# ShuvalovIvan/RayTracingProject

Hardware: AMD Instinct MI355X
Metric: Mrays/sec + frame time, random-spheres 1920x1080x256spp (higher is better)
Workload: dtype f32

## Files before the change

### raytracingproject_amd/build.py

```python
from __future__ import annotations

import os
import subprocess
from concurrent.futures import ThreadPoolExecutor
from pathlib import Path

PKG = Path(__file__).resolve().parent
ROOT = PKG.parent
CSRC = PKG / "csrc"
OBJ = PKG / "build"
LIB = PKG / "lib" / "librt_hip.so"
ARCH = os.environ.get("RT_OFFLOAD_ARCH", "gfx950")
HIPCC = os.environ.get("HIPCC", "/opt/rocm/bin/hipcc")

COMMON = ["-x", "hip", f"--offload-arch={ARCH}", "-O3", "-std=c++17", "-fPIC", "-Wall",
          "-Wno-unused-function", f"-I{ROOT / 'include'}"] + os.environ.get("RT_HIPCC_EXTRA", "").split()
UNITS = {
    "rt_render_f32.hip": ["-fno-hip-fp32-correctly-rounded-divide-sqrt", "-fgpu-flush-denormals-to-zero",
                          os.environ.get("RT_F32_CONTRACT", "-ffp-contract=on")],
    "rt_render_f64.hip": ["-ffp-contract=off"],
    "rt_abi.cpp": ["-ffp-contract=off"],
    "rt_plan.cpp": ["-ffp-contract=off"],
    "rt_pack.cpp": ["-ffp-contract=off"],
    "rt_bvh.cpp": ["-ffp-contract=off"],
    "rt_obj.cpp": ["-ffp-contract=off"],
    "rt_lbvh.hip": ["-ffp-contract=off"],
    "rt_comm.cpp": [],
}
HEADERS = ["rt_device.h", "rt_render_impl.h", "rt_occluded.h", "rt_scene.h", "rt_launch.h", "rt_bvh.h", "rt_lbvh.h", "rt_ctx.h",
           "rt_treelet.h", "rt_pack.h"]


def _stale(target: Path, deps: list[Path]) -> bool:
    if not target.exists():
        return True
    t = target.stat().st_mtime
    return any(d.stat().st_mtime > t for d in deps)


def _present(p: Path) -> bool:
    try:
        return p.exists()
    except OSError:
        return False


def _compile(src: str, extra: list[str], verbose: bool) -> Path:
    obj = OBJ / (src.rsplit(".", 1)[0] + ".o")
    deps = [CSRC / src] + [CSRC / h for h in HEADERS] + [ROOT / "include" / "rt_hip.h", Path(__file__)]
    if _stale(obj, deps):
        cmd = [HIPCC, *COMMON, *extra, "-c", str(CSRC / src), "-o", str(obj)]
        if verbose:
            print(" ".join(cmd), flush=True)
        subprocess.run(cmd, check=True)
    return obj


def build_native(verbose: bool = False) -> Path:
    OBJ.mkdir(parents=True, exist_ok=True)
    LIB.parent.mkdir(parents=True, exist_ok=True)
    with ThreadPoolExecutor(max_workers=4) as ex:
        objs = list(ex.map(lambda kv: _compile(kv[0], kv[1], verbose), UNITS.items()))
    if _stale(LIB, objs):
# ... 82 lines not shown
BOXES_EXE = OBJ / "san" / "bvh_boxes_driver"


def build_bvh_boxes(verbose: bool = False) -> Path:
    BOXES_EXE.parent.mkdir(parents=True, exist_ok=True)
    srcs = [ROOT / "tests" / "cpp" / "bvh_boxes_driver.cpp", CSRC / "rt_bvh.cpp"]
    deps = srcs + [CSRC / "rt_bvh.h", CSRC / "rt_scene.h", ROOT / "include" / "rt_hip.h", Path(__file__)]
    if _stale(BOXES_EXE, deps):
        cmd = ["g++", "-std=c++17", *SAN_FLAGS, "-ffp-contract=off", f"-I{ROOT / 'include'}", *map(str, srcs), "-o",
               str(BOXES_EXE), "-lm"]
        if verbose:
            print(" ".join(cmd), flush=True)
        subprocess.run(cmd, check=True)
    return BOXES_EXE


PACK_EXE = OBJ / "san" / "pack_driver"


def build_pack(verbose: bool = False) -> Path:
    PACK_EXE.parent.mkdir(parents=True, exist_ok=True)
    srcs = [ROOT / "tests" / "cpp" / "pack_driver.cpp", CSRC / "rt_pack.cpp", CSRC / "rt_bvh.cpp"]
    deps = srcs + [CSRC / "rt_pack.h", CSRC / "rt_bvh.h", CSRC / "rt_scene.h", ROOT / "include" / "rt_hip.h",
                   Path(__file__)]
    if _stale(PACK_EXE, deps):
        cmd = ["g++", "-std=c++17", *SAN_FLAGS, "-ffp-contract=off", f"-I{ROOT / 'include'}", *map(str, srcs), "-o",
               str(PACK_EXE), "-lm"]
        if verbose:
            print(" ".join(cmd), flush=True)
        subprocess.run(cmd, check=True)
    return PACK_EXE


def build_oracle(verbose: bool = False) -> None:
    oracle = ROOT / "oracle"
    out = None if verbose else subprocess.DEVNULL
    subprocess.run(["make", "-C", str(oracle), "liboracle.so", "rt_oracle_cli", "ref-if-present"], check=True,
                   stdout=out)


if __name__ == "__main__":
    import sys
    if "--sanitize" in sys.argv[1:]:
        print(build_sanitize(verbose=True))
        sys.exit(0)
    print(build_native(verbose=True))
    print(build_dropin(verbose=True))
    build_oracle(verbose=True)
```

### raytracingproject_amd/csrc/rt_abi.cpp

```cpp
#include <hip/hip_runtime.h>

#include <algorithm>
#include <array>
#include <cmath>
#include <cstdarg>
#include <limits>
#include <cstdio>
#include <cstdlib>
#include <cstring>
#include <string>
#include <vector>

#include "../../include/rt_hip.h"
#include "rt_bvh.h"
#include "rt_device.h"
#include "rt_launch.h"
#include "rt_lbvh.h"
#include "rt_ctx.h"

using namespace rtx;
using namespace rtx_abi;


namespace {
// ... 104 lines not shown
    int n = 0;
    if (hipGetDeviceCount(&n) != hipSuccess) return 0;
    return n;
}

const char* rt_error_string(int code) {
    switch (code) {
        case RT_OK: return "ok";
        case RT_ERR_INVALID: return "invalid argument";
        case RT_ERR_HIP: return "HIP runtime error";
        case RT_ERR_NO_SCENE: return "no scene uploaded";
        case RT_ERR_LIMIT: return "scene or image exceeds kernel limits";
        case RT_ERR_COMM: return "RCCL error";
        default: return "unknown error";
    }
}

static bool parse_grid_suspend(const char* s, int& lanes, int& iters) {
    if (!s || !*s) return true;
    int l = 0, i = 0, n = 0;
    if (sscanf(s, "%d,%d%n", &l, &i, &n) == 2 && !s[n] && l >= 1 && l <= 64 && i >= 1 && i <= 65535) {
        lanes = l;
        iters = i;
        return true;
    }
    if (s[0] == '0' && !s[1]) {
        lanes = 0;
        iters = 0x7fffffff;
        return true;
    }
    return false;
}

rt_ctx* rt_create(int device, uint64_t seed, int precision) {
    if (precision != RT_PREC_F32 && precision != RT_PREC_F64) return nullptr;
    int n = 0;
    if (hipGetDeviceCount(&n) != hipSuccess || device < 0 || device >= n) return nullptr;
    if (hipSetDevice(device) != hipSuccess) return nullptr;
    rt_ctx* c = new rt_ctx();
    if (!parse_grid_suspend(getenv("RT_GRID_SUSPEND"), c->gsus_lanes, c->gsus_iters)) {
        fprintf(stderr, "rt_create: RT_GRID_SUSPEND must be \"0\" or \"LANES,ITERS\" (1..64, 1..65535)\n");
        delete c;
        return nullptr;
    }
    c->device = device;
    c->seed = seed;
    c->precision = precision;
    if (hipDeviceGetAttribute(&c->n_cu, hipDeviceAttributeMultiprocessorCount, device) != hipSuccess) c->n_cu = 0;
    if (hipStreamCreateWithFlags(&c->stream, hipStreamNonBlocking) != hipSuccess ||
        hipEventCreate(&c->ev0) != hipSuccess || hipEventCreate(&c->ev1) != hipSuccess ||
        hipMalloc((void**)&c->d_small, 16 * sizeof(double)) != hipSuccess ||
        hipMalloc((void**)&c->d_used, sizeof(int)) != hipSuccess) {
        rt_destroy(c);
        return nullptr;
    }
    return c;
}

void rt_destroy(rt_ctx* c) {
    if (!c) return;
    (void)hipSetDevice(c->device);
    if (c->stream) (void)hipStreamSynchronize(c->stream);
    free_scene(c);
    (void)hipFree(c->d_shard);
    (void)hipFree(c->d_frame);
    (void)hipFree(c->d_segs);
    (void)hipFree(c->d_segs_frame);
    (void)hipFree(c->d_rgb);
    (void)hipFree(c->d_tape);
    (void)hipFree(c->d_small);
    (void)hipFree(c->d_used);
    (void)hipFree(c->d_samples);
    (void)hipFree(c->d_queue64);
    (void)hipFree(c->d_gather);
// ... 362 lines not shown
}

static int launch_rc(rt_ctx* c, hipError_t e) {
    return e == hipSuccess ? RT_OK : fail(c, RT_ERR_HIP, "render launch: %s", hipGetErrorString(e));
}

static int render_range_f32(rt_ctx* c, const LaunchPlan& plan, RenderParams P, size_t npx, hipStream_t st) {
    float* out_sums = (float*)P.out_sums;
    int rc;
    rt_ctx::Accum* slot = nullptr;
    for (auto& a : c->accum)
        if (a.out == out_sums && a.W == P.W && a.H == P.H && a.shard == P.shard && a.nshards == P.nshards) slot = &a;
    const bool have = slot != nullptr;
    if (!slot) {
        slot = &c->accum[0];
        for (auto& a : c->accum)
            if (a.used < slot->used) slot = &a;
    }
    if ((rc = grow(c, (void**)&slot->acc, &slot->acc_cap, npx * 3 * sizeof(long long)))) return rc;
    if ((rc = grow(c, (void**)&slot->accp, &slot->accp_cap, npx * 2 * sizeof(unsigned long long)))) return rc;
    if ((rc = grow(c, (void**)&slot->flags, &slot->flags_cap, npx * sizeof(uint32_t)))) return rc;
    slot->out = out_sums;
    slot->W = P.W;
    slot->H = P.H;
    slot->shard = P.shard;
    slot->nshards = P.nshards;
    slot->used = ++c->accum_clock;
    P.accum = slot->acc;
    P.accum_flags = slot->flags;
    P.accp = slot->accp;
    P.diag = c->diag_buf;
    P.gsus_lanes = c->gsus_lanes;
    P.gsus_iters = c->gsus_iters;
    if (!slot->queue) HIPCHK(c, hipMalloc((void**)&slot->queue, QUEUE_CTRL_BYTES));
    P.queue = slot->queue;
    {
        const double lanes = (double)P.max_wgs * plan.block, pixels = (double)npx;
        plan_phases(P, P.spp, lanes, pixels, item_balance_of(c, lanes, pixels), item_cap(c, plan.trav, lanes, pixels));
    }
    HIPCHK(c, hipMemsetAsync(slot->queue, 0, QUEUE_CTRL_BYTES, st));
    HIPCHK(c, hipMemsetAsync(slot->accp, 0, npx * 2 * sizeof(unsigned long long), st));
    hipError_t e = hipSuccess;
    if (!P.accumulate) {
        e = hipMemsetAsync(slot->acc, 0, npx * 3 * sizeof(long long), st);
        if (e == hipSuccess) e = hipMemsetAsync(slot->flags, 0, npx * sizeof(uint32_t), st);
        if (e == hipSuccess && P.out_segs) e = hipMemsetAsync(P.out_segs, 0, npx * sizeof(uint32_t), st);
    } else if (!have) {
        e = launch_seed_accum(out_sums, slot->acc, slot->flags, npx, st);
    } else {
        e = launch_reconcile_accum(out_sums, slot->acc, slot->flags, npx, st);
    }
    if (e == hipSuccess && P.spp > 0)
        e = c->diag_buf ? launch_render_f32_diag(P, plan.lds_bytes, st, plan.trav, plan.block, plan.wpe)
                        : launch_render_f32(P, plan.lds_bytes, st, plan.block, plan.wpe, plan.trav);
    if (e == hipSuccess) e = launch_finalize(slot->acc, slot->accp, slot->flags, out_sums, npx, st);
    return launch_rc(c, e);
}

static int render_range_f64(rt_ctx* c, const LaunchPlan& plan, const RenderParams& P, size_t npx, hipStream_t st) {
    const int spp = P.spp;
    const size_t eb = elem_bytes(c);
    int rc;
    constexpr size_t MAX_PASS_SAMPLES = 0xffff;
    const size_t fit = std::min(MAX_PASS_SAMPLES, npx > 0 ? ((size_t)c->tuning.sample_buffer_mb << 20) /
                                                                (npx * 3 * eb) : (size_t)spp);
    const int pass_spp = std::max(1, (size_t)spp < fit ? spp : (int)std::max<size_t>(1, fit));
// ... 401 lines not shown
```

### raytracingproject_amd/csrc/rt_ctx.h

```cpp
#pragma once
#include <hip/hip_runtime.h>

#include <cstdarg>
#include <cstdint>
#include <cstdio>
#include <array>
#include <string>
#include <vector>

#include "../../include/rt_hip.h"
#include "rt_device.h"
#include "rt_lbvh.h"
#include "rt_pack.h"

using namespace rtx;

struct rt_ctx {
    int device = 0;
    int precision = RT_PREC_F32;
    uint64_t seed = 0;
    hipStream_t stream = nullptr;
    hipEvent_t ev0 = nullptr, ev1 = nullptr;
    bool timed = false;
    std::string err;
    rt_tuning tuning{1024, 6, 1.0, 0.25, 8, RT_TRAV_DEFAULT, 2, -1, 2.0, 65536, 16384, RT_MESH_BUILD_HOST, -1, -1, 0, 32, 8.0, 20.0, 48, 0, 0, -1, 2.0, 32};

    bool has_scene = false;
    Node* d_nodes = nullptr;
    void* d_sph = nullptr;
    void* d_mat = nullptr;
    SphereD* d_big = nullptr;
    BigF* d_bigf = nullptr;
    int n_nodes = 0, n_sph = 0, n_mat = 0, n_big = 0, depth = 0, leaves = 0, n_input = 0;
    int n_front = 0;
    float box_extent = 0.f;
    void* d_grid = nullptr;
    int grid_nodes = 0;
    GridHdr grid_hdr{};
    int grid_entries = 0;
    double grid_density = 0.0;
    SceneReach reach;
    int gsus_lanes = GSUS_DEFAULT_LANES, gsus_iters = GSUS_DEFAULT_ITERS;
    int* d_remap = nullptr;
    int* d_unmap = nullptr;
    int n_unmap = 0;
    Node4* d_mnodes = nullptr;
    void* d_tris = nullptr;
    uint32_t* d_tmeta = nullptr;
    int n_mnodes = 0, n_tris = 0, mdepth = 0, mleaves = 0;
    float mbox[6] = {};
    LbvhScratch lbvh;

    void* d_shard = nullptr;
    size_t shard_cap = 0;
    void* d_frame = nullptr;
    size_t frame_cap = 0;
    uint32_t* d_segs = nullptr;
    size_t segs_cap = 0;
    uint32_t* d_segs_frame = nullptr;
    size_t segs_frame_cap = 0;
    int32_t* d_rgb = nullptr;
    size_t rgb_cap = 0;
    double* d_tape = nullptr;
    size_t tape_cap = 0;
    double* d_small = nullptr;
    int* d_used = nullptr;
    void* d_samples = nullptr;
    uint32_t* d_queue64 = nullptr;
    size_t samples_cap = 0;
    void* d_gather = nullptr;
    size_t gather_cap = 0;

    struct Accum {
        const void* out = nullptr;
        int W = 0, H = 0, shard = 0, nshards = 0;
// ... 67 lines not shown
```

### raytracingproject_amd/csrc/rt_device.h

```cpp
#pragma once
#include <type_traits>
#include <hip/hip_runtime.h>

#include <cstdint>

#include "rt_scene.h"


namespace rtx {

__host__ __device__ __forceinline__ uint32_t hash32(uint32_t x) {
    x ^= x >> 16;
    x *= 0x21f0aaadu;
    x ^= x >> 15;
    x *= 0xd35a2d97u;
    x ^= x >> 15;
    return x;
}
__host__ __device__ __forceinline__ uint32_t seed32_of(uint64_t seed) {
    return hash32((uint32_t)seed ^ hash32((uint32_t)(seed >> 32)));
}
constexpr uint32_t RNG_GOLDEN = 0x9e3779b9u;
constexpr uint32_t RNG_SAMPLE_SALT = 0x85ebca6bu;

struct CounterRng {
    uint32_t st;
    __device__ __forceinline__ void start(uint32_t pixel_key, uint32_t sample) {
        st = hash32(pixel_key ^ hash32(sample ^ RNG_SAMPLE_SALT));
    }
    template <class R>
    __device__ __forceinline__ R next() {
        st += RNG_GOLDEN;
        return (R)(hash32(st) >> 8) * (R)(1.0 / 16777216.0);
    }
    template <class R>
    __device__ __forceinline__ R next_affine(R s, R c) {
        st += RNG_GOLDEN;
        return fma((R)(hash32(st) >> 8), s * (R)(1.0 / 16777216.0), c);
    }
// ... 67 lines not shown
    int n_nodes, n_spheres, n_mats, n_big;
    int n_front;
    int stack_size;
    int defocus;
    double cam_center[3], p00[3], du[3], dv[3], ddu[3], ddv[3];
    float f_center[3], f_p00[3], f_du[3], f_dv[3], f_ddu[3], f_ddv[3];
    const Node* nodes;
    const void* spheres;
    const void* mats;
    const SphereD* big;
    const BigF* bigf;
    const Node4* mnodes;
    const void* tris;
    const uint32_t* tmeta;
    int n_mnodes;
    int mstack;
    void* out_sums;
    uint32_t* out_segs;
    unsigned long long* diag;
    void* samples;
    long long* accum;
    uint32_t* accum_flags;
    unsigned long long* accp;
    uint32_t* queue;
    int max_wgs;
    int nph;
    int ph_s0[MAX_PHASES], ph_c[MAX_PHASES], ph_k[MAX_PHASES];
    int coh_refill;
    float box_extent;
    float mbox[6];
    GridHdr grid;
    double tiles_x_inv, tiles_x_inv_half;
    int gsus_lanes, gsus_iters;
};
constexpr int GSUS_DEFAULT_LANES = 16, GSUS_DEFAULT_ITERS = 8;
constexpr size_t QUEUE_CTRL_BYTES = 4096;
constexpr int FIX_SHIFT = 28;
constexpr int FIX_SAMPLE_SHIFT = 19;
constexpr int FIX_ITEM_SAMPLES = 32;
constexpr int FIX_LAUNCH_SAMPLES = 8191;
constexpr uint32_t FIX_NAN = 1u, FIX_POS = 2u, FIX_NEG = 4u;
constexpr int DIAG_SLOTS = 32;

constexpr int COH_FIFO = 128;
template <bool MESH>
struct CohEntryT {
    float t;
    uint32_t pix;
    uint32_t sid;
};
template <>
struct CohEntryT<true> {
    float t;
    uint32_t pix;
    uint32_t sid;
    int32_t id;
};
using CohEntry = CohEntryT<false>;
static_assert(sizeof(CohEntryT<false>) == 12 && sizeof(CohEntryT<true>) == 16, "CohEntry");
template <bool MESH>
struct CohEntryD {
    double t;
    uint32_t pix;
    uint32_t sid;
};
template <>
struct CohEntryD<true> {
    double t;
    uint32_t pix;
    uint32_t sid;
    int32_t id;
    uint32_t pad;
};
static_assert(sizeof(CohEntryD<false>) == 16 && sizeof(CohEntryD<true>) == 24, "CohEntryD");
template <class R, bool MESH> struct CohEntrySel { using type = CohEntryT<MESH>; };
template <bool MESH> struct CohEntrySel<double, MESH> { using type = CohEntryD<MESH>; };
template <class R, bool MESH> using CohEntryX = typename CohEntrySel<R, MESH>::type;
constexpr size_t COH_SUM_BYTES = 64 * 3 * sizeof(float);
constexpr size_t COH_PARK_BYTES = 64 * 4 * sizeof(float);
constexpr size_t coh_wave_bytes(bool mesh, bool sums, int fifo = COH_FIFO, bool f64 = false, bool park = false) {
    return (size_t)fifo * (f64 ? (mesh ? sizeof(CohEntryD<true>) : sizeof(CohEntryD<false>))
                               : (mesh ? sizeof(CohEntryT<true>) : sizeof(CohEntryT<false>))) +
           (sums && !f64 ? COH_SUM_BYTES : 0) + (park ? COH_PARK_BYTES : 0);
}
constexpr size_t COH_WAVE_BYTES = coh_wave_bytes(false, true);
struct CohConst {
    float cam[18];
    int nph;
    int ph_s0[MAX_PHASES], ph_c[MAX_PHASES], ph_k[MAX_PHASES];
    int pad;
};
static_assert(sizeof(CohConst) % 16 == 0, "CohConst");
constexpr size_t COH_CAM_BYTES = sizeof(CohConst);


template <class R> struct Prec;
template <> struct Prec<float> { using Sph = SphereF; using Mat = MatF; using Tri = TriF; };
template <> struct Prec<double> { using Sph = SphereD; using Mat = MatD; using Tri = TriD; };

template <class R>
struct SceneView {
    const Node* nodes;
    const typename Prec<R>::Sph* sph;
    const typename Prec<R>::Mat* mat;
    const SphereD* big;
    const BigF* bigf;
    int n_nodes, n_big, n_front;
    const Node4* mnodes;
    const typename Prec<R>::Tri* tris;
    const uint32_t* tmeta;
    int n_mnodes;
    uint32_t* mstack;
    int n_mstack;
    float mbox[6];
    GridHdr grid;
    const __attribute__((address_space(4))) GridHdr* gridp;
// ... 172 lines not shown
            s.clo[a] = -__builtin_huge_valf();
            s.chi[a] = __builtin_huge_valf();
            continue;
        }
        const float f = (float)(1.0 / dd[a]);
        const float m = (float)((fabs(oo[a]) + (double)extent) * 0x1p-21 * fabs((double)f));
        const float c = -((float)oo[a] * f);
        s.f[a] = f;
        s.clo[a] = f > 0.f ? c - m : c + m;
        s.chi[a] = f > 0.f ? c + m : c - m;
    }
    return s;
}
__device__ __forceinline__ bool box_hit_cons(const float lo[3], const float hi[3], const ConsSlabs& s, float tmin,
                                             float tmax, float& tnear) {
    const float t0x = __builtin_fmaf(lo[0], s.f[0], s.clo[0]), t1x = __builtin_fmaf(hi[0], s.f[0], s.chi[0]);
    const float t0y = __builtin_fmaf(lo[1], s.f[1], s.clo[1]), t1y = __builtin_fmaf(hi[1], s.f[1], s.chi[1]);
    const float t0z = __builtin_fmaf(lo[2], s.f[2], s.clo[2]), t1z = __builtin_fmaf(hi[2], s.f[2], s.chi[2]);
    const float tn = fmaxf(fmaxf(fminf(t0x, t1x), fminf(t0y, t1y)), fmaxf(fminf(t0z, t1z), tmin));
    const float tf = fminf(fminf(fmaxf(t0x, t1x), fmaxf(t0y, t1y)), fmaxf(t0z, t1z));
    tnear = tn;
    return tn <= tf && tn <= tmax;
}
constexpr float CONS_TMIN = 0.0009f;
__device__ __forceinline__ float cons_tmax(double tmax) { return (float)tmax * (1.f + 0x1p-22f); }

enum { TRAV_SELROOT = 8, TRAV_B128 = 16, TRAV_F32BOX = 32, TRAV_COH = 64, TRAV_NOSUM = 128, TRAV_TBIN = 256,
       TRAV_CULL = 512, TRAV_PERSIST = 2048, TRAV_MTOP = 4096, TRAV_MIFIF = 8192, TRAV_MWHILE = 16384,
       TRAV_MQ = 32768, TRAV_GRID = 65536, TRAV_GFLAT = 131072,
       TRAV_G3D = 262144 };
constexpr int TRAV_REMOVED = TRAV_TBIN | TRAV_MTOP;
constexpr int coh_fifo_entries(int) { return COH_FIFO; }
constexpr bool coh_parks(bool mesh, int tr, bool f64) { return mesh && !f64 && (tr & TRAV_GRID) != 0; }
typedef __attribute__((address_space(3))) const uint32_t lds_cu32;
typedef __attribute__((address_space(3))) const float4 lds_cf4;
__device__ __forceinline__ void keep_live(uint32_t v) { asm volatile("" ::"v"(v)); }
template <class R, bool EXACT, bool DIAG = false, int TRAV = 0, bool MESH = false, bool SUSP = false>
__device__ __forceinline__ Hit<R> closest_hit(const SceneView<R>& sc, const Ray<R>& ray, uint16_t* stack, int stride,
                                              int self_id, DiagCounters* dg = nullptr, float* resume = nullptr,
                                              const Hit<R>* part = nullptr, int sus_lanes = 0, int sus_iters = 0) {
    static_assert(!SUSP || (!EXACT && !MESH && (TRAV & TRAV_GRID) != 0 && (TRAV & TRAV_GFLAT) != 0),
                  "resumable walks: the fp32 sphere-only flat grid walk");
    constexpr R TMIN = (R)0.001;
    Hit<R> h;
    h.id = -1;
    h.td = __builtin_huge_val();
    R tmax = (R)__builtin_huge_valf();
    const V3<R> o = ray.o, d = ray.d;
    const R a = len2(d);
    const R inv_a = rcp(a);
    [[maybe_unused]] bool resumed = false;
    [[maybe_unused]] float t_from = -1.f;
    if constexpr (SUSP) {
        t_from = *resume;
        *resume = -1.f;
        resumed = t_from >= 0.f;
        if (resumed) {
            h.id = part->id;
            tmax = part->t;
        }
    }

    if (SUSP && resumed) {
    } else if (EXACT) {
        const V3<double> od = cvt<double>(o), dd = cvt<double>(d);
        double tmaxd = __builtin_huge_val();
        for (int k = 0; k < sc.n_big; ++k) {
            const SphereD& s = sc.big[k];
            double t;
            if (sphere_root<double, true>(mk(s.c[0], s.c[1], s.c[2]), s.r, mk(s.cv[0], s.cv[1], s.cv[2]),
                                          (s.meta >> 30) & 1u, od, dd, (double)a, 0.0, (double)ray.time, 0.001,
                                          tmaxd, false, t)) {
                tmaxd = t;
                h.id = -2 - k;
                h.td = t;
// ... 16 lines not shown
                const R disc = b * b - a * cc;
                if (disc < 0) continue;
                const R qq = b + copysign((R)sqrt(disc), b);
                const R ta = cc * rcp(qq), tb = qq * inv_a;
                const R t0 = fmin(ta, tb), t1 = fmax(ta, tb);
                t = t0;
                if (!(TMIN < t && t < tmax)) {
                    t = t1;
                    if (!(TMIN < t && t < tmax)) continue;
                }
            }
            tmax = t;
            h.id = -2 - k;
        }
    }

    using Sph = typename Prec<R>::Sph;
    auto test_rec = [&](const Sph* rec, bool is_self, R tlim, R& tk) -> bool {
        if constexpr (!EXACT && (TRAV & TRAV_B128) != 0) {
            const float4* q = (const float4*)rec;
            const float4 s0 = q[0], s1 = q[1];
            keep_live(__float_as_uint(s0.w));
            keep_live(__float_as_uint(s1.w));
            return sphere_root<R, false, (TRAV & TRAV_SELROOT) != 0>(
                mk((R)s0.x, (R)s0.y, (R)s0.z), (R)s0.w, mk((R)s1.x, (R)s1.y, (R)s1.z), false, o, d, a, inv_a,
                ray.time, TMIN, tlim, is_self, tk);
        }
        const auto& s = *rec;
        return sphere_root<R, EXACT, (TRAV & TRAV_SELROOT) != 0>(mk((R)s.c[0], (R)s.c[1], (R)s.c[2]), (R)s.r,
                                     mk((R)s.cv[0], (R)s.cv[1], (R)s.cv[2]), (s.meta >> 30) & 1u, o, d, a, inv_a,
                                     ray.time, TMIN, tlim, !EXACT && is_self, tk);
    };
    auto test_one = [&](int k, R tlim, R& tk) -> bool { return test_rec(sc.sph + k, k == self_id, tlim, tk); };
    for (int k = 0; k < (SUSP && resumed ? 0 : sc.n_front); ++k) {
        R t;
        if (test_one(k, tmax, t)) {
            tmax = t;
            h.id = k;
        }
    }

    if constexpr ((TRAV & TRAV_GRID) != 0) {
        if (sc.n_nodes > 0) {
            constexpr bool FLAT = (TRAV & TRAV_GFLAT) != 0;
            const GridHdr g = [&]() {
                if constexpr (!MESH) {
                    auto gp = sc.gridp;
                    asm volatile("" : "+s"(gp));
                    return *(const GridHdr*)gp;
                } else {
                    return sc.grid;
                }
            }();
            const uint32_t pad = (uint32_t)g.res[0] * (uint32_t)g.res[1];
            const uint32_t* cells = (const uint32_t*)sc.nodes + pad;
            const unsigned char* lbase = (const unsigned char*)sc.nodes;
            const uint32_t sph0 = (uint32_t)sc.n_nodes * (uint32_t)sizeof(Node);
            const uint32_t self_off = self_id >= 0 && self_id < MESH_HIT_BASE
                                          ? sph0 + (uint32_t)self_id * (uint32_t)sizeof(Sph)
                                          : 0xffffffffu;
            uint32_t hit_off = 0xffffffffu;
            const float INF = __builtin_huge_valf();
            const V3<float> of = cvt<float>(o), df = cvt<float>(d);
            float tn, tf, nx, ny = INF, nz, dtx, dty = 0.f, dtz;
            int ci;
            {
// ... 575 lines not shown
```

### raytracingproject_amd/csrc/rt_plan.cpp

```cpp
#include <algorithm>
#include <array>
#include <map>
#include <mutex>

#include "rt_ctx.h"
#include "rt_launch.h"

using namespace rtx;

namespace rtx_abi {

int stack_entries(const rt_ctx* c) { return c->depth > 1 ? c->depth - 1 : 1; }

size_t lds_scene_bytes_at(const rt_ctx* c, int block, int tr) {
    const bool grid = (tr & TRAV_GRID) != 0;
    const size_t sph = c->precision == RT_PREC_F64 ? sizeof(SphereD) : sizeof(SphereF);
    const size_t mat = c->precision == RT_PREC_F64 ? sizeof(MatD) : sizeof(MatF);
    const size_t stack = grid ? 0 : (size_t)block * (size_t)stack_entries(c) * 2;
    return (size_t)(grid ? c->grid_nodes : c->n_nodes) * sizeof(Node) + (size_t)c->n_sph * sph +
           (size_t)c->n_mat * mat + (size_t)c->n_big * (sizeof(SphereD) + sizeof(BigF)) + ((stack + 15) & ~(size_t)15);
}


namespace {
// ... 5 lines not shown
                                       : std::array<int, 6>{0, mesh, block, wpe, tr, 0};
    {
        std::lock_guard<std::mutex> g(mu);
        const auto it = known.find(key);
        if (it != known.end()) return it->second;
    }
    const int v = f64 ? render_f64_vgprs(mesh, f64k) : render_f32_vgprs(block, wpe, tr, mesh);
    if (v > 0) {
        std::lock_guard<std::mutex> g(mu);
        known[key] = v;
    }
    return v;
}

struct Planner {
    const rt_ctx* c;
    bool grid_usable;

    bool grid_flat() const {
        return grid_usable && c->grid_hdr.res[1] == 1 && !(c->tuning.traversal & TRAV_G3D);
    }
    int f64_kernel_of() const {
        const int k = c->tuning.f64_kernel > 0 ? c->tuning.f64_kernel
                      : (c->tuning.traversal & TRAV_GRID) ? F64_KERNEL_GRID : F64_KERNEL_DEFAULT;
        if (k != F64_KERNEL_GRID) return k;
        return !grid_usable ? F64_KERNEL_DEFAULT : grid_flat() ? F64_KERNEL_GRID_FLAT : k;
    }

    size_t lds_sphere_bytes_bt(int block, int tr) const {
        const bool f32 = c->precision == RT_PREC_F32;
        const size_t nw = (size_t)(block / 64);
        const size_t coh = c->n_mnodes > 0 || !(tr & TRAV_COH)
                               ? 0
                               : nw * coh_wave_bytes(false, (tr & TRAV_NOSUM) == 0, coh_fifo_entries(tr), !f32) + COH_CAM_BYTES;
        return lds_scene_bytes_at(c, block, tr) + coh;
    }

    size_t lds_mesh_bytes_at(int block, int tr, int s) const {
        if (c->n_mnodes == 0) return 0;
        const size_t stack = (size_t)block * (size_t)s * 4;
        const bool f64 = c->precision != RT_PREC_F32;
        if (tr & TRAV_COH)
            return stack +
                   (size_t)(block / 64) *
                       coh_wave_bytes(true, (tr & TRAV_NOSUM) == 0, coh_fifo_entries(tr), f64, coh_parks(true, tr, f64)) +
                   COH_CAM_BYTES;
        if (f64) return stack;
        return stack + (size_t)block * 3 * sizeof(float);
    }

    int wgs_per_cu_bt(int block, int tr, int wpe) const {
        const bool mesh = c->n_mnodes > 0;
        const int v = kernel_vgprs(c->precision == RT_PREC_F64, mesh, block, wpe, tr, f64_kernel_of());
        int waves = v > 0 ? 512 / ((v + 7) & ~7) : 8;
        if (waves > 8) waves = 8;
        const int wgs = waves * 4 / (block / 64);
        return wgs > 0 ? wgs : 1;
    }

    int occupancy_at(int block, int tr, int wpe, int s) const {
        const int reg = wgs_per_cu_bt(block, tr, wpe);
        const size_t need = lds_sphere_bytes_bt(block, tr) + lds_mesh_bytes_at(block, tr, s);
        const int lds = need > 0 ? (int)(160 * 1024 / need) : 64;
        return reg < lds ? reg : lds;
    }

    static constexpr int MESH_LDS_STACK_AUTO = 12;
    int mesh_stack_bt(int block, int tr, int wpe) const {
        if (c->n_mnodes == 0) return 0;
        if (c->tuning.mesh_lds_stack >= 0) return c->tuning.mesh_lds_stack;
        if (tr & TRAV_GRID) return 0;
        const int most = occupancy_at(block, tr, wpe, 0);
        for (int s = MESH_LDS_STACK_AUTO; s > 0; --s)
            if (occupancy_at(block, tr, wpe, s) >= most) return s;
        return 0;
    }

    int occupancy_bt(int block, int tr, int wpe) const {
        return occupancy_at(block, tr, wpe, mesh_stack_bt(block, tr, wpe));
    }

    LaunchPlan plan_of() const {
        int t = c->tuning.traversal;
        if (c->precision != RT_PREC_F32 || c->n_mnodes == 0) t &= ~TRAV_MIFIF;
        const bool want_mifif = (t & TRAV_MIFIF) || !(t & TRAV_MWHILE);
        t &= ~(TRAV_MWHILE | TRAV_MIFIF | TRAV_GFLAT | TRAV_G3D);
        if (c->precision == RT_PREC_F64)
            return {render_f64_block(f64_kernel_of()), render_f64_trav(f64_kernel_of()), 0};
        if (!grid_usable) t &= ~TRAV_GRID;
        const bool flat = grid_flat();
        auto gflat = [&](int b, int w, int x, bool mesh) {
            return flat && (x & TRAV_GRID) && render_f32_supported(b, w, x | TRAV_GFLAT, mesh) ? x | TRAV_GFLAT : x;
        };
        if (c->n_mnodes == 0) {
            const int b = c->tuning.block, w = c->tuning.waves_per_eu;
            if ((t & TRAV_COH) && !(t & TRAV_NOSUM)) {
                const size_t base = lds_scene_bytes_at(c, b, t), nw = (size_t)(b / 64);
                const int fifo = coh_fifo_entries(t);
                const size_t with = base + nw * coh_wave_bytes(false, true, fifo) + COH_CAM_BYTES,
                             without = base + nw * coh_wave_bytes(false, false, fifo) + COH_CAM_BYTES;
                const int reg = wgs_per_cu_bt(b, t, w);
                if (std::min<size_t>(reg, 160 * 1024 / with) < std::min<size_t>(reg, 160 * 1024 / without))
                    t |= TRAV_NOSUM;
            }
            return {b, gflat(b, w, t, false), w};
        }
        if (!(t & TRAV_COH)) t &= ~TRAV_NOSUM;
        const int wt = c->tuning.mesh_waves_per_eu;
        const int t0 = t;
        LaunchPlan cand[12];
        int nc = 0;
        for (int b : {256, 512, 768}) {
            if (c->tuning.mesh_block > 0 && b != c->tuning.mesh_block) continue;
            const int ws[2] = {wt >= 0 ? wt : 0, 6};
            for (int wi = 0; wi < (wt >= 0 ? 1 : 2); ++wi)
            for (int gi = 0; gi < ((t & TRAV_GRID) ? 2 : 1); ++gi) {
                const int w = ws[wi];
                const int t = gi ? t0 & ~TRAV_GRID : t0;
                auto mifif = [&](int x) {
                    return want_mifif && render_f32_supported(b, w, x | TRAV_MIFIF, true) ? x | TRAV_MIFIF : x;
                };
                int tb = mifif(t);
                if ((t & TRAV_COH) && !(t & TRAV_NOSUM)) {
                    const int tn = mifif(t | TRAV_NOSUM);
                    const bool ok_with = render_f32_supported(b, w, tb, true);
                    const bool ok_without = render_f32_supported(b, w, tn, true);
                    if (!ok_with || (ok_without && occupancy_bt(b, tb, w) < occupancy_bt(b, tn, w))) tb = tn;
                }
                if (render_f32_supported(b, w, tb, true)) cand[nc++] = {b, gflat(b, w, tb, true), w};
            }
        }
        bool any_mifif = false;
        for (int i = 0; i < nc; ++i) any_mifif = any_mifif || (cand[i].trav & TRAV_MIFIF) != 0;
// ... 33 lines not shown
```

### raytracingproject_amd/csrc/rt_render_impl.h

```cpp
#pragma once
#include "rt_device.h"
#include "rt_launch.h"

namespace rtx {

__device__ __forceinline__ V3<float> mul_rn(V3<float> a, V3<float> b) {
#pragma clang fp contract(off)
    return {a.x * b.x, a.y * b.y, a.z * b.z};
}
__device__ __forceinline__ V3<float> add_rn(V3<float> a, V3<float> b) {
#pragma clang fp contract(off)
    return {a.x + b.x, a.y + b.y, a.z + b.z};
}
__device__ __forceinline__ V3<double> mul_rn(V3<double> a, V3<double> b) { return a * b; }
__device__ __forceinline__ V3<double> add_rn(V3<double> a, V3<double> b) { return a + b; }

__device__ __forceinline__ void copy16(void* dst, const void* src, size_t bytes, int tid, int nthreads) {
    uint4* d = (uint4*)dst;
    const uint4* s = (const uint4*)src;
    const size_t n = bytes / 16;
    for (size_t k = (size_t)tid; k < n; k += (size_t)nthreads) d[k] = s[k];
}

constexpr uint32_t ITEM_NONE = 0xffffffffu;
// ... 316 lines not shown

template <class R, bool EXACT, int BLOCK, int TRAV, bool MESH, bool DIAG = false>
__device__ __forceinline__ void render_coherent(const RenderParams& P0, const SceneView<R>& sc, uint16_t* stack,
                                                CohEntryX<R, MESH>* fifo, float* isum, const CohConst& kc) {
    static_assert(!EXACT || (sizeof(R) == 8 && !DIAG), "EXACT: fp64, no instrumented build");
    constexpr bool LAUNDER = !MESH || (TRAV & TRAV_GRID) != 0;
    typedef __attribute__((address_space(4))) const RenderParams KArg;
    auto kernarg = []() {
        KArg* p = (KArg*)__builtin_amdgcn_kernarg_segment_ptr();
        if constexpr (LAUNDER) asm volatile("" : "+s"(p));
        return p;
    };
    [[maybe_unused]] KArg* Pp = kernarg();
#define P (LAUNDER ? *(const RenderParams*)Pp : P0)
    const float* cam = kc.cam;
    constexpr float SC = (float)(1 << FIX_SAMPLE_SHIFT), ISC = 1.f / SC;
    constexpr int TR = TRAV & ~(TRAV_COH | TRAV_NOSUM | TRAV_PERSIST);
    constexpr bool SUMS = !EXACT && (TRAV & TRAV_NOSUM) == 0;
    [[maybe_unused]] R* const samp = (R*)P.samples;
    [[maybe_unused]] const size_t npx_all = (size_t)P.shard_tiles * 64;
#ifndef RT_KDEF_MESH
#define RT_KDEF_MESH 1
#endif
    constexpr bool KDEF = !EXACT && (!MESH || (RT_KDEF_MESH && (TRAV & TRAV_GRID) != 0));
    static_assert(MAX_LEAF_FIRST + MAX_BIG + 16 <= 0xfff, "sphere hit id + 16 must fit sid bits 16-27");
    auto cam_ray = [&](int px, int py, CounterRng& rr, int kdef = -1, int* kout = nullptr) -> Ray<R> {
        if constexpr (EXACT)
            return camera_ray<R>(P, px, py, rr);
        else
            return camera_ray_lds(cam, P.defocus, px, py, rr, kdef, kout);
    };
    constexpr int FIFO = coh_fifo_entries(TRAV);
    const int lane = threadIdx.x & 63;
    DiagCounters dg, dgb;
    unsigned long long n_bounce = 0, n_live = 0, cyc_trav = 0, cyc_shade = 0, cyc_batch = 0, n_paths = 0, n_seg = 0,
                       n_batch = 0, n_pop = 0;
    const unsigned long long t_start = DIAG ? __builtin_amdgcn_s_memtime() : 0;
    const unsigned long long rt_start = DIAG ? __builtin_amdgcn_s_memrealtime() : 0;
    unsigned long long rt_dry = 0, n_drain = 0;
    unsigned long long n_in_item = 0, n_direct = 0, n_item_flush = 0;

    uint32_t head = 0, count = 0;
    ItemDec cur = decode_item(P, P, ITEM_NONE);
    int bi = 0;
    bool dry = false;
    if (SUMS) isum[lane] = isum[64 + lane] = isum[128 + lane] = 0.f;

    bool elig = false;
    auto finish = [&](uint32_t pp, bool in_item, V3<R> L, uint32_t sg, uint32_t srel) {
        if constexpr (EXACT) {
            R* o = samp + ((size_t)srel * npx_all + pp) * 3;
            o[0] = L.x;
            o[1] = L.y;
            o[2] = L.z;
            if (P.out_segs && sg) atomicAdd(P.out_segs + pp, sg);
            return;
        }
        const float qx = __builtin_rintf(L.x * SC) * ISC, qy = __builtin_rintf(L.y * SC) * ISC,
                    qz = __builtin_rintf(L.z * SC) * ISC;
        const bool in01 = qx >= 0.f && qx <= 1.f && qy >= 0.f && qy <= 1.f && qz >= 0.f && qz <= 1.f;
        if (SUMS && in_item && in01) {
            const uint32_t q = pp & 63u;
            if (qx != 0.f) atomicAdd(isum + q, qx);
            if (qy != 0.f) atomicAdd(isum + 64 + q, qy);
            if (qz != 0.f) atomicAdd(isum + 128 + q, qz);
            if (P.out_segs && sg) atomicAdd(P.out_segs + pp, sg);
            if (DIAG) ++n_in_item;
        } else {
            flush_sample(P, pp, qx, qy, qz, sg);
            if (DIAG) ++n_direct;
        }
        if (DIAG) ++n_paths;
    };

    auto batch = [&]() {
        const unsigned long long tb = DIAG ? __builtin_amdgcn_s_memtime() : 0;
        if (bi >= cur.c) {
            if (SUMS && cur.lt >= 0) {
                const float fx = isum[lane], fy = isum[64 + lane], fz = isum[128 + lane];
                if (fx != 0.f || fy != 0.f || fz != 0.f) {
                    flush_sample(P, (uint32_t)cur.lt * 64u + (uint32_t)lane, fx, fy, fz, 0u, (float)cur.c);
                    if (DIAG) ++n_item_flush;
                }
                isum[lane] = isum[64 + lane] = isum[128 + lane] = 0.f;
            }
            cur = decode_item(P, kc, fetch_item(P, kc));
            bi = 0;
            elig = false;
            if (cur.lt < 0) {
                dry = true;
                if (DIAG) rt_dry = __builtin_amdgcn_s_memrealtime();
                return;
            }
        }
        const int s = cur.s0 + bi++;
        const int px = cur.tx0 + (lane & 7), py = cur.ty0 + (lane >> 3);
        const uint32_t pp = (uint32_t)cur.lt * 64u + (uint32_t)lane;
        bool hit = false;
        Hit<R> hb;
        hb.t = (R)0;
        hb.id = -1;
        [[maybe_unused]] int kd = 15;
        if (px < P.W && py < P.H && P.max_depth > 0) {
            CounterRng r2;
            r2.start(hash32(P.seed32 ^ (uint32_t)(py * P.W + px)), (uint32_t)s);
            const Ray<R> pr = KDEF ? cam_ray(px, py, r2, -1, &kd) : cam_ray(px, py, r2);
            hb = closest_hit<R, EXACT, DIAG, TR, MESH>(sc, pr, stack, BLOCK, NO_SELF, &dgb);
            if (hb.id == -1) {
                finish(pp, true, sky(pr.d), 1u, (uint32_t)(s - P.sample_begin));
            } else {
                hit = true;
            }
        } else if constexpr (EXACT) {
            finish(pp, true, mk((R)0, (R)0, (R)0), 0u, (uint32_t)(s - P.sample_begin));
        }
        const unsigned long long hm = __ballot(hit);
        if (hit) {
            const uint32_t r = __builtin_amdgcn_mbcnt_hi((uint32_t)(hm >> 32), __builtin_amdgcn_mbcnt_lo((uint32_t)hm, 0u));
            CohEntryX<R, MESH> e;
            e.t = hb.t;
            e.pix = pp;
            if constexpr (MESH) {
                e.sid = (uint32_t)(s - P.sample_begin);
                if constexpr (KDEF) e.sid |= (uint32_t)min(kd, 15) << 28;
                e.id = hb.id;
            } else {
                e.sid = (uint32_t)(s - P.sample_begin) | ((uint32_t)(hb.id + 16) << 16);
                if constexpr (KDEF) e.sid |= (uint32_t)min(kd, 15) << 28;
            }
            fifo[(head + count + r) & (FIFO - 1)] = e;
        }
        count += (uint32_t)__popcll(hm);
        if (DIAG && lane == 0) {
            ++n_batch;
            cyc_batch += __builtin_amdgcn_s_memtime() - tb;
        }
    };

    bool live = false, ready = false, fin = false;
    constexpr bool SUSP = !EXACT && !MESH && (TR & TRAV_GRID) != 0 && (TR & TRAV_GFLAT) != 0;
// ... 253 lines not shown
    static_assert(!EXACT || sizeof(R) == 8, "EXACT needs fp64");
    extern __shared__ __attribute__((aligned(16))) unsigned char smem[];

    using Sph = typename Prec<R>::Sph;
    using Mat = typename Prec<R>::Mat;
    const size_t nb_nodes = (size_t)P.n_nodes * sizeof(Node);
    const size_t nb_sph = (size_t)P.n_spheres * sizeof(Sph);
    const size_t nb_mat = (size_t)P.n_mats * sizeof(Mat);
    const size_t nb_big = (size_t)P.n_big * sizeof(SphereD);
    const size_t nb_bigf = (size_t)P.n_big * sizeof(BigF);
    unsigned char* base = smem;
    Node* s_nodes = (Node*)base;
    base += nb_nodes;
    Sph* s_sph = (Sph*)base;
    base += nb_sph;
    Mat* s_mat = (Mat*)base;
    base += nb_mat;
    SphereD* s_big = (SphereD*)base;
    base += nb_big;
    BigF* s_bigf = (BigF*)base;
    base += nb_bigf;
    uint16_t* s_stack = (uint16_t*)base;
    base += ((size_t)BLOCK * (size_t)P.stack_size * 2 + 15) & ~(size_t)15;
    uint32_t* s_mstack = (uint32_t*)base;

    const int tid = threadIdx.x;
    copy16(s_nodes, P.nodes, nb_nodes, tid, BLOCK);
    copy16(s_sph, P.spheres, nb_sph, tid, BLOCK);
    copy16(s_mat, P.mats, nb_mat, tid, BLOCK);
    copy16(s_big, P.big, nb_big, tid, BLOCK);
    copy16(s_bigf, P.bigf, nb_bigf, tid, BLOCK);
    if constexpr ((TRAV & TRAV_COH) != 0) {
        constexpr size_t WB =
            coh_wave_bytes(MESH, (TRAV & TRAV_NOSUM) == 0, coh_fifo_entries(TRAV), EXACT, coh_parks(MESH, TRAV, EXACT));
        CohConst* kc = (CohConst*)((unsigned char*)(s_mstack + (size_t)BLOCK * P.mstack) + (size_t)(BLOCK / 64) * WB);
        if (tid == 0) {
#pragma unroll
            for (int k = 0; k < 3; ++k) {
                kc->cam[k] = P.f_center[k];
                kc->cam[3 + k] = P.f_p00[k];
                kc->cam[6 + k] = P.f_du[k];
                kc->cam[9 + k] = P.f_dv[k];
                kc->cam[12 + k] = P.f_ddu[k];
                kc->cam[15 + k] = P.f_ddv[k];
            }
            kc->nph = P.nph;
#pragma unroll
            for (int k = 0; k < MAX_PHASES; ++k) {
                kc->ph_s0[k] = P.ph_s0[k];
                kc->ph_c[k] = P.ph_c[k];
                kc->ph_k[k] = P.ph_k[k];
            }
        }
    }
    __syncthreads();

    SceneView<R> sc;
    sc.nodes = s_nodes;
    sc.sph = s_sph;
    sc.mat = s_mat;
    sc.big = s_big;
    sc.bigf = s_bigf;
    sc.n_nodes = P.n_nodes;
    sc.n_big = P.n_big;
    sc.n_front = P.n_front;
    sc.mnodes = P.mnodes;
    sc.tris = (const typename Prec<R>::Tri*)P.tris;
    sc.tmeta = P.tmeta;
    sc.n_mnodes = MESH ? P.n_mnodes : 0;
    sc.mstack = s_mstack + tid;
    sc.n_mstack = MESH ? P.mstack : 0;
    sc.box_extent = P.box_extent;
    for (int a = 0; a < 6; ++a) sc.mbox[a] = P.mbox[a];
    sc.grid = P.grid;
    sc.gridp = (const __attribute__((address_space(4))) GridHdr*)((const __attribute__((address_space(4))) char*)
                                                                       __builtin_amdgcn_kernarg_segment_ptr() +
                                                                   offsetof(RenderParams, grid));
    uint16_t* stack = s_stack + tid;
    if constexpr ((TRAV & TRAV_COH) != 0) {
        constexpr size_t WB =
            coh_wave_bytes(MESH, (TRAV & TRAV_NOSUM) == 0, coh_fifo_entries(TRAV), EXACT, coh_parks(MESH, TRAV, EXACT));
        unsigned char* r0 = (unsigned char*)(s_mstack + (size_t)BLOCK * P.mstack);
        unsigned char* w = r0 + (size_t)(tid >> 6) * WB;
        const CohConst* kc = (const CohConst*)(r0 + (size_t)(BLOCK / 64) * WB);
        render_coherent<R, EXACT, BLOCK, TRAV, MESH, DIAG>(
            P, sc, stack, (CohEntryX<R, MESH>*)w, (float*)(w + coh_fifo_entries(TRAV) * sizeof(CohEntryX<R, MESH>)),
            *kc);
    } else if constexpr (!EXACT) {
        render_lanes<R, BLOCK, TRAV, MESH, DIAG>(P, sc, stack, (float*)(s_mstack + (size_t)BLOCK * P.mstack) + tid);
    } else {
        static_assert(!EXACT || (TRAV & TRAV_PERSIST) != 0, "fp64 kernels run on persistent lanes");
        render_lanes<R, BLOCK, TRAV, MESH, false, true>(P, sc, stack, nullptr);
    }
}

struct TraceHit {
    double t, p[3], normal[3];
    int32_t id, front_face, mat, pad;
};
static_assert(sizeof(TraceHit) == 72, "rt_hit");

template <class R, bool EXACT, int BLOCK, int TRAV, bool MESH, bool DIAG = false>
__global__ __launch_bounds__(BLOCK) void trace_kernel(RenderParams P, const R* __restrict__ rays, int n,
                                                      TraceHit* __restrict__ hits, const int* __restrict__ remap,
                                                      const int* __restrict__ origin_ids,
                                                      const int* __restrict__ unmap, int n_unmap) {
    extern __shared__ __attribute__((aligned(16))) unsigned char smem[];
    uint16_t* s_stack;
    uint32_t* s_mstack;
    const SceneView<R> sc = load_scene_lds<R, BLOCK, TRAV, MESH>(P, smem, s_stack, s_mstack);
    __syncthreads();
    uint16_t* stack = s_stack + threadIdx.x;
    DiagCounters dg;
    for (int base = blockIdx.x * BLOCK; base < n; base += gridDim.x * BLOCK) {
// ... 156 lines not shown
```

Baseline: 17790.

## Cull spheres per 8x8 camera tile into wave candidate list for primary rays

For the fp32 sphere-grid coherent kernels, each wave builds a conservative beam around its 8x8 pixel tile when it starts a new tile batch. It culls all spheres against that beam with a ballot and compacts, storing up to 24 surviving sphere offsets in a per-wave LDS list. Primary rays then test only those candidates instead of walking the grid, falling back to the normal traversal when too many survive. This adds a per-tile O(N spheres) culling pass and extra LDS per wave, which may lower occupancy. For random-spheres with many spheres, the fallback may fire often.

```diff
diff --git a/raytracingproject_amd/build.py b/raytracingproject_amd/build.py
--- a/raytracingproject_amd/build.py
+++ b/raytracingproject_amd/build.py
@@ -28,7 +28,7 @@
     "rt_comm.cpp": [],
 }
 HEADERS = ["rt_device.h", "rt_render_impl.h", "rt_occluded.h", "rt_scene.h", "rt_launch.h", "rt_bvh.h", "rt_lbvh.h", "rt_ctx.h",
-           "rt_treelet.h", "rt_pack.h"]
+           "rt_treelet.h", "rt_pack.h", "rt_batch_cull.h"]
 
 
 def _stale(target: Path, deps: list[Path]) -> bool:
@@ -177,6 +177,29 @@
     return PACK_EXE
 
 
+CULL_EXE = OBJ / "san" / "batch_cull_driver"
+CULL_MUTANTS = (1, 2, 3)
+
+
+def build_batch_cull(verbose: bool = False) -> list[Path]:
+    CULL_EXE.parent.mkdir(parents=True, exist_ok=True)
+    src = ROOT / "tests" / "cpp" / "batch_cull_driver.cpp"
+    deps = [src, CSRC / "rt_batch_cull.h", CSRC / "rt_scene.h", Path(__file__)]
+    exes = [CULL_EXE] + [CULL_EXE.with_name(f"batch_cull_driver_m{m}") for m in CULL_MUTANTS]
+
+    def one(k: int) -> None:
+        if _stale(exes[k], deps):
+            cmd = ["g++", "-std=c++17", *SAN_FLAGS, "-O2", "-ffp-contract=off", f"-DRT_CULL_MUTATE={k}", f"-I{CSRC}", str(src),
+                   "-o", str(exes[k]), "-lm"]
+            if verbose:
+                print(" ".join(cmd), flush=True)
+            subprocess.run(cmd, check=True)
+
+    with ThreadPoolExecutor(max_workers=4) as ex:
+        list(ex.map(one, range(len(exes))))
+    return exes
+
+
 def build_oracle(verbose: bool = False) -> None:
     oracle = ROOT / "oracle"
     out = None if verbose else subprocess.DEVNULL
diff --git a/raytracingproject_amd/csrc/rt_abi.cpp b/raytracingproject_amd/csrc/rt_abi.cpp
--- a/raytracingproject_amd/csrc/rt_abi.cpp
+++ b/raytracingproject_amd/csrc/rt_abi.cpp
@@ -160,6 +160,16 @@
     return false;
 }
 
+static bool parse_batch_cull(const char* s, int& cap) {
+    if (!s || !*s) return true;
+    int v = 0, n = 0;
+    if (sscanf(s, "%d%n", &v, &n) == 1 && !s[n] && v >= 0 && v <= BATCH_CAND_CAP) {
+        cap = v;
+        return true;
+    }
+    return false;
+}
+
 rt_ctx* rt_create(int device, uint64_t seed, int precision) {
     if (precision != RT_PREC_F32 && precision != RT_PREC_F64) return nullptr;
     int n = 0;
@@ -168,6 +178,11 @@
     rt_ctx* c = new rt_ctx();
     if (!parse_grid_suspend(getenv("RT_GRID_SUSPEND"), c->gsus_lanes, c->gsus_iters)) {
         fprintf(stderr, "rt_create: RT_GRID_SUSPEND must be \"0\" or \"LANES,ITERS\" (1..64, 1..65535)\n");
+        delete c;
+        return nullptr;
+    }
+    if (!parse_batch_cull(getenv("RT_BATCH_CULL"), c->batch_cap)) {
+        fprintf(stderr, "rt_create: RT_BATCH_CULL must be 0..%d\n", BATCH_CAND_CAP);
         delete c;
         return nullptr;
     }
@@ -596,6 +611,8 @@
     P.diag = c->diag_buf;
     P.gsus_lanes = c->gsus_lanes;
     P.gsus_iters = c->gsus_iters;
+    P.batch_cap = c->batch_cap;
+    P.batch_pad = 0;
     if (!slot->queue) HIPCHK(c, hipMalloc((void**)&slot->queue, QUEUE_CTRL_BYTES));
     P.queue = slot->queue;
     {
diff --git a/raytracingproject_amd/csrc/rt_batch_cull.h b/raytracingproject_amd/csrc/rt_batch_cull.h
--- /dev/null
+++ b/raytracingproject_amd/csrc/rt_batch_cull.h
@@ -0,0 +1,80 @@
+#pragma once
+#include <cmath>
+#include <cstddef>
+#include <cstdint>
+
+#include "rt_scene.h"
+
+namespace rtx {
+
+constexpr int BATCH_CAND_CAP = 24;
+constexpr size_t BATCH_CAND_BYTES = 128;
+static_assert((BATCH_CAND_CAP + 1) * 4 <= BATCH_CAND_BYTES, "candidate list");
+
+#ifndef RT_CULL_MUTATE
+#define RT_CULL_MUTATE 0
+#endif
+#if RT_CULL_MUTATE == 1
+constexpr float CULL_EPS = 0x1p-29f, CULL_EPS_CAM = 0x1p-31f, CULL_UP = 1.f;
+#else
+constexpr float CULL_EPS = 0x1p-17f, CULL_EPS_CAM = 0x1p-19f, CULL_UP = 1.f + 0x1p-19f;
+#endif
+
+struct CullBeam {
+    float c[3], ax[3];
+    float rl, g, scale;
+    bool ok;
+};
+
+RT_HD inline CullBeam cull_beam(const float* cam, int defocus, int tx0, int ty0) {
+    auto nrm = [](const float* v) { return sqrtf(v[0] * v[0] + v[1] * v[1] + v[2] * v[2]); };
+    auto l1 = [](const float* v) { return fabsf(v[0]) + fabsf(v[1]) + fabsf(v[2]); };
+    const float* c = cam;
+    const float *p00 = cam + 3, *du = cam + 6, *dv = cam + 9, *ddu = cam + 12, *ddv = cam + 15;
+    const float fx = (float)tx0 + 3.5f, fy = (float)ty0 + 3.5f;
+    CullBeam b;
+    float a[3];
+    for (int k = 0; k < 3; ++k) {
+        b.c[k] = c[k];
+        a[k] = (p00[k] + fx * du[k] + fy * dv[k]) - c[k];
+    }
+    const float L = nrm(a);
+    const float iL = 1.f / L;
+    for (int k = 0; k < 3; ++k) b.ax[k] = a[k] * iL;
+    b.scale = l1(c) + l1(p00) + (fx + 4.5f) * l1(du) + (fy + 4.5f) * l1(dv) + l1(ddu) + l1(ddv);
+    const float E = CULL_EPS_CAM * b.scale;
+    const float rho = 4.f * (nrm(du) + nrm(dv)) * CULL_UP + E;
+#if RT_CULL_MUTATE == 2
+    b.rl = E;
+#else
+    b.rl = (defocus ? nrm(ddu) + nrm(ddv) : 0.f) * CULL_UP + E;
+#endif
+    const float k = (b.rl + rho) * iL * CULL_UP;
+    b.ok = k <= 0.875f;
+    b.g = k / (1.f - k) * CULL_UP * CULL_UP;
+    return b;
+}
+
+RT_HD inline bool cull_keep(const CullBeam& b, const SphereF& s) {
+    const float hx = 0.5f * s.cv[0], hy = 0.5f * s.cv[1], hz = 0.5f * s.cv[2];
+#if RT_CULL_MUTATE == 3
+    const float rb = fabsf(s.r);
+#else
+    const float rb = fabsf(s.r) + sqrtf(hx * hx + hy * hy + hz * hz) * CULL_UP;
+#endif
+    const float qx = (s.c[0] + hx) - b.c[0], qy = (s.c[1] + hy) - b.c[1], qz = (s.c[2] + hz) - b.c[2];
+    const float qn = sqrtf(qx * qx + qy * qy + qz * qz);
+    const float sa = qx * b.ax[0] + qy * b.ax[1] + qz * b.ax[2];
+    const float px = qx - sa * b.ax[0], py = qy - sa * b.ax[1], pz = qz - sa * b.ax[2];
+    const float perp = sqrtf(px * px + py * py + pz * pz);
+    const float W = (rb + b.rl) + CULL_EPS * (qn + b.scale + rb);
+    const float bound = (W + b.g * fmaxf(sa + W, 0.f)) * CULL_UP;
+    const bool behind = sa < -W, outside = perp > bound;
+    return !b.ok || !(behind || outside);
+}
+
+RT_HD inline bool batch_cull_keep(const float* cam, int defocus, int tx0, int ty0, const SphereF& s) {
+    return cull_keep(cull_beam(cam, defocus, tx0, ty0), s);
+}
+
+}
diff --git a/raytracingproject_amd/csrc/rt_ctx.h b/raytracingproject_amd/csrc/rt_ctx.h
--- a/raytracingproject_amd/csrc/rt_ctx.h
+++ b/raytracingproject_amd/csrc/rt_ctx.h
@@ -41,6 +41,7 @@
     double grid_density = 0.0;
     SceneReach reach;
     int gsus_lanes = GSUS_DEFAULT_LANES, gsus_iters = GSUS_DEFAULT_ITERS;
+    int batch_cap = BATCH_CAND_CAP;
     int* d_remap = nullptr;
     int* d_unmap = nullptr;
     int n_unmap = 0;
diff --git a/raytracingproject_amd/csrc/rt_device.h b/raytracingproject_amd/csrc/rt_device.h
--- a/raytracingproject_amd/csrc/rt_device.h
+++ b/raytracingproject_amd/csrc/rt_device.h
@@ -5,6 +5,7 @@
 #include <cstdint>
 
 #include "rt_scene.h"
+#include "rt_batch_cull.h"
 
 
 namespace rtx {
@@ -138,6 +139,7 @@
     GridHdr grid;
     double tiles_x_inv, tiles_x_inv_half;
     int gsus_lanes, gsus_iters;
+    int batch_cap, batch_pad;
 };
 constexpr int GSUS_DEFAULT_LANES = 16, GSUS_DEFAULT_ITERS = 8;
 constexpr size_t QUEUE_CTRL_BYTES = 4096;
@@ -184,10 +186,11 @@
 template <class R, bool MESH> using CohEntryX = typename CohEntrySel<R, MESH>::type;
 constexpr size_t COH_SUM_BYTES = 64 * 3 * sizeof(float);
 constexpr size_t COH_PARK_BYTES = 64 * 4 * sizeof(float);
-constexpr size_t coh_wave_bytes(bool mesh, bool sums, int fifo = COH_FIFO, bool f64 = false, bool park = false) {
+constexpr size_t coh_wave_bytes(bool mesh, bool sums, int fifo = COH_FIFO, bool f64 = false, bool park = false,
+                                bool cand = false) {
     return (size_t)fifo * (f64 ? (mesh ? sizeof(CohEntryD<true>) : sizeof(CohEntryD<false>))
                                : (mesh ? sizeof(CohEntryT<true>) : sizeof(CohEntryT<false>))) +
-           (sums && !f64 ? COH_SUM_BYTES : 0) + (park ? COH_PARK_BYTES : 0);
+           (sums && !f64 ? COH_SUM_BYTES : 0) + (park ? COH_PARK_BYTES : 0) + (cand ? BATCH_CAND_BYTES : 0);
 }
 constexpr size_t COH_WAVE_BYTES = coh_wave_bytes(false, true);
 struct CohConst {
@@ -426,15 +429,19 @@
 constexpr int TRAV_REMOVED = TRAV_TBIN | TRAV_MTOP;
 constexpr int coh_fifo_entries(int) { return COH_FIFO; }
 constexpr bool coh_parks(bool mesh, int tr, bool f64) { return mesh && !f64 && (tr & TRAV_GRID) != 0; }
+constexpr bool coh_cands(bool mesh, int tr, bool f64) { return !mesh && !f64 && (tr & TRAV_GRID) != 0; }
 typedef __attribute__((address_space(3))) const uint32_t lds_cu32;
 typedef __attribute__((address_space(3))) const float4 lds_cf4;
 __device__ __forceinline__ void keep_live(uint32_t v) { asm volatile("" ::"v"(v)); }
-template <class R, bool EXACT, bool DIAG = false, int TRAV = 0, bool MESH = false, bool SUSP = false>
+template <class R, bool EXACT, bool DIAG = false, int TRAV = 0, bool MESH = false, bool SUSP = false,
+          bool CAND = false>
 __device__ __forceinline__ Hit<R> closest_hit(const SceneView<R>& sc, const Ray<R>& ray, uint16_t* stack, int stride,
                                               int self_id, DiagCounters* dg = nullptr, float* resume = nullptr,
-                                              const Hit<R>* part = nullptr, int sus_lanes = 0, int sus_iters = 0) {
+                                              const Hit<R>* part = nullptr, int sus_lanes = 0, int sus_iters = 0,
+                                              uint32_t clist = 0, int ncand = 0) {
     static_assert(!SUSP || (!EXACT && !MESH && (TRAV & TRAV_GRID) != 0 && (TRAV & TRAV_GFLAT) != 0),
                   "resumable walks: the fp32 sphere-only flat grid walk");
+    static_assert(!CAND || (!SUSP && coh_cands(MESH, TRAV, EXACT)), "candidate lists: the fp32 sphere-grid kernels");
     constexpr R TMIN = (R)0.001;
     Hit<R> h;
     h.id = -1;
@@ -517,6 +524,24 @@
                                      ray.time, TMIN, tlim, !EXACT && is_self, tk);
     };
     auto test_one = [&](int k, R tlim, R& tk) -> bool { return test_rec(sc.sph + k, k == self_id, tlim, tk); };
+    if constexpr (CAND) {
+        uint32_t hit_off = 0xffffffffu;
+        for (int i = 0; i < ncand; ++i) {
+            if (DIAG) DiagCounters::count(dg->leaf_it, dg->leaf_act), ++dg->steps;
+            const uint32_t off = (uint32_t)__builtin_amdgcn_readfirstlane(
+                (int)*(const lds_cu32*)(uintptr_t)(clist + 4u * (uint32_t)i));
+            const Sph* rec = (const Sph*)(const float4*)(const lds_cf4*)(uintptr_t)off;
+            R t;
+            if (test_rec(rec, false, tmax, t)) {
+                tmax = t;
+                hit_off = off;
+            }
+        }
+        if (hit_off != 0xffffffffu)
+            h.id = (int)((hit_off - (uint32_t)sc.n_nodes * (uint32_t)sizeof(Node)) / (uint32_t)sizeof(Sph));
+        h.t = tmax;
+        return h;
+    }
     for (int k = 0; k < (SUSP && resumed ? 0 : sc.n_front); ++k) {
         R t;
         if (test_one(k, tmax, t)) {
diff --git a/raytracingproject_amd/csrc/rt_plan.cpp b/raytracingproject_amd/csrc/rt_plan.cpp
--- a/raytracingproject_amd/csrc/rt_plan.cpp
+++ b/raytracingproject_amd/csrc/rt_plan.cpp
@@ -61,7 +61,9 @@
         const size_t nw = (size_t)(block / 64);
         const size_t coh = c->n_mnodes > 0 || !(tr & TRAV_COH)
                                ? 0
-                               : nw * coh_wave_bytes(false, (tr & TRAV_NOSUM) == 0, coh_fifo_entries(tr), !f32) + COH_CAM_BYTES;
+                               : nw * coh_wave_bytes(false, (tr & TRAV_NOSUM) == 0, coh_fifo_entries(tr), !f32, false,
+                                                    coh_cands(false, tr, !f32)) +
+                                     COH_CAM_BYTES;
         return lds_scene_bytes_at(c, block, tr) + coh;
     }
 
@@ -126,8 +128,9 @@
             if ((t & TRAV_COH) && !(t & TRAV_NOSUM)) {
                 const size_t base = lds_scene_bytes_at(c, b, t), nw = (size_t)(b / 64);
                 const int fifo = coh_fifo_entries(t);
-                const size_t with = base + nw * coh_wave_bytes(false, true, fifo) + COH_CAM_BYTES,
-                             without = base + nw * coh_wave_bytes(false, false, fifo) + COH_CAM_BYTES;
+                const bool cand = coh_cands(false, t, false);
+                const size_t with = base + nw * coh_wave_bytes(false, true, fifo, false, false, cand) + COH_CAM_BYTES,
+                             without = base + nw * coh_wave_bytes(false, false, fifo, false, false, cand) + COH_CAM_BYTES;
                 const int reg = wgs_per_cu_bt(b, t, w);
                 if (std::min<size_t>(reg, 160 * 1024 / with) < std::min<size_t>(reg, 160 * 1024 / without))
                     t |= TRAV_NOSUM;
diff --git a/raytracingproject_amd/csrc/rt_render_impl.h b/raytracingproject_amd/csrc/rt_render_impl.h
--- a/raytracingproject_amd/csrc/rt_render_impl.h
+++ b/raytracingproject_amd/csrc/rt_render_impl.h
@@ -372,6 +372,9 @@
     };
     constexpr int FIFO = coh_fifo_entries(TRAV);
     const int lane = threadIdx.x & 63;
+    constexpr bool CAND = coh_cands(MESH, TRAV, EXACT);
+    [[maybe_unused]] uint32_t* const clist =
+        (uint32_t*)((unsigned char*)fifo + (size_t)FIFO * sizeof(CohEntryX<R, MESH>) + (SUMS ? COH_SUM_BYTES : 0));
     DiagCounters dg, dgb;
     unsigned long long n_bounce = 0, n_live = 0, cyc_trav = 0, cyc_shade = 0, cyc_batch = 0, n_paths = 0, n_seg = 0,
                        n_batch = 0, n_pop = 0;
@@ -432,6 +435,28 @@
                 if (DIAG) rt_dry = __builtin_amdgcn_s_memrealtime();
                 return;
             }
+            if constexpr (CAND) {
+                const int cap = P.batch_cap;
+                uint32_t n = 0xffffffffu;
+                if (cap > 0) {
+                    const CullBeam bm = cull_beam(cam, P.defocus, cur.tx0, cur.ty0);
+                    const int nsph = P.n_spheres;
+                    const uint32_t sph0 = (uint32_t)sc.n_nodes * (uint32_t)sizeof(Node);
+                    n = 0;
+                    for (int b0 = 0; b0 < nsph; b0 += 64) {
+                        const int k = b0 + lane;
+                        const bool keep = k < nsph && cull_keep(bm, sc.sph[k]);
+                        const unsigned long long km = __ballot(keep);
+                        const uint32_t r = n + __builtin_amdgcn_mbcnt_hi((uint32_t)(km >> 32),
+                                                                         __builtin_amdgcn_mbcnt_lo((uint32_t)km, 0u));
+                        if (keep && r < (uint32_t)BATCH_CAND_CAP) clist[r] = sph0 + (uint32_t)k * (uint32_t)sizeof(SphereF);
+                        n += (uint32_t)__popcll(km);
+                    }
+                    if (n > (uint32_t)cap) n = 0xffffffffu;
+                }
+                if (lane == 0) clist[BATCH_CAND_CAP] = n;
+                __builtin_amdgcn_wave_barrier();
+            }
         }
         const int s = cur.s0 + bi++;
         const int px = cur.tx0 + (lane & 7), py = cur.ty0 + (lane >> 3);
@@ -445,7 +470,16 @@
             CounterRng r2;
             r2.start(hash32(P.seed32 ^ (uint32_t)(py * P.W + px)), (uint32_t)s);
             const Ray<R> pr = KDEF ? cam_ray(px, py, r2, -1, &kd) : cam_ray(px, py, r2);
-            hb = closest_hit<R, EXACT, DIAG, TR, MESH>(sc, pr, stack, BLOCK, NO_SELF, &dgb);
+            if constexpr (CAND) {
+                const int nc = __builtin_amdgcn_readfirstlane((int)clist[BATCH_CAND_CAP]);
+                if (nc >= 0)
+                    hb = closest_hit<R, EXACT, DIAG, TR, MESH, false, true>(sc, pr, stack, BLOCK, NO_SELF, &dgb, nullptr,
+                                                                            nullptr, 0, 0, (uint32_t)(uintptr_t)clist, nc);
+                else
+                    hb = closest_hit<R, EXACT, DIAG, TR, MESH>(sc, pr, stack, BLOCK, NO_SELF, &dgb);
+            } else {
+                hb = closest_hit<R, EXACT, DIAG, TR, MESH>(sc, pr, stack, BLOCK, NO_SELF, &dgb);
+            }
             if (hb.id == -1) {
                 finish(pp, true, sky(pr.d), 1u, (uint32_t)(s - P.sample_begin));
             } else {
@@ -765,7 +799,8 @@
     copy16(s_bigf, P.bigf, nb_bigf, tid, BLOCK);
     if constexpr ((TRAV & TRAV_COH) != 0) {
         constexpr size_t WB =
-            coh_wave_bytes(MESH, (TRAV & TRAV_NOSUM) == 0, coh_fifo_entries(TRAV), EXACT, coh_parks(MESH, TRAV, EXACT));
+            coh_wave_bytes(MESH, (TRAV & TRAV_NOSUM) == 0, coh_fifo_entries(TRAV), EXACT, coh_parks(MESH, TRAV, EXACT),
+                           coh_cands(MESH, TRAV, EXACT));
         CohConst* kc = (CohConst*)((unsigned char*)(s_mstack + (size_t)BLOCK * P.mstack) + (size_t)(BLOCK / 64) * WB);
         if (tid == 0) {
 #pragma unroll
@@ -812,7 +847,8 @@
     uint16_t* stack = s_stack + tid;
     if constexpr ((TRAV & TRAV_COH) != 0) {
         constexpr size_t WB =
-            coh_wave_bytes(MESH, (TRAV & TRAV_NOSUM) == 0, coh_fifo_entries(TRAV), EXACT, coh_parks(MESH, TRAV, EXACT));
+            coh_wave_bytes(MESH, (TRAV & TRAV_NOSUM) == 0, coh_fifo_entries(TRAV), EXACT, coh_parks(MESH, TRAV, EXACT),
+                           coh_cands(MESH, TRAV, EXACT));
         unsigned char* r0 = (unsigned char*)(s_mstack + (size_t)BLOCK * P.mstack);
         unsigned char* w = r0 + (size_t)(tid >> 6) * WB;
         const CohConst* kc = (const CohConst*)(r0 + (size_t)(BLOCK / 64) * WB);
```

Result: faster. 19150 (median of 6 runs) (+7.6%).
